# iamarkaj/AwesomeSLAM

Measured on AMD Instinct MI355X. Metric: EKF/UKF filter-steps/s @ N_landmarks, higher is better.
Workload: dtype f32

## Files before the change

### awesomeslam_amd/csrc/aslam_core.hip

```cpp
#include "../../include/aslam_core.h"
#include "../../include/aslam_scan.h"
#include "../../include/aslam_snapshot.h"

#include <hip/hip_runtime.h>

#include <cmath>
#include <cstdio>
#include <cstring>
#include <cstdlib>
#include <algorithm>
#include <mutex>
#include <string>
#include <type_traits>
#include <vector>

#include "ekf_small.h"
#include "ekf_large.h"
#include "ekf_large_launch.h"
#include "scan_front.h"
#include "snapshot.h"
#if ASLAM_HAVE_UKF
#include "ukf_small.h"
#include "ukf_large.h"
#include "ukf_large_launch.h"
// ... 1355 lines not shown
        if (chol_resident)
                *chol_resident = c->large && c->lh.last_resident;
        if (launches_per_callback)
                *launches_per_callback = c->large ? c->lh.last_launches : 1;
        return ASLAM_OK;
}

int aslam_kernel_info(aslam_ctx *c, char *name, int name_cap, int *grid, int *block, int *lds_bytes)
{
        if (!c)
                return fail(ASLAM_ERR_ARG, "null context");
        char buf[192];
        size_t lds = 0;
        if (c->large)
        {
                const LargePlan plan = large_plan(c->cfg.dtype == ASLAM_F32, c->NP, c->cfg.batch, c->cfg.batch, c->lh.knobs);
#if ASLAM_HAVE_UKF
                if (c->cfg.filter == ASLAM_UKF)
                        std::snprintf(buf, sizeof(buf), "ukf_large_wabt + large_update_panel<double> + large_syrk<double> (%d-launch chain per callback, 1 stream)",
                                      ukf_large_plan(c->NP).launches);
                else
#endif
                if (plan.chain == LargeChain::F32_RESIDENT)
                        std::snprintf(buf, sizeof(buf), "%s + %s + large_syrk_bf16x3 (%d-launch chain per callback, %d stream groups)",
                                      plan.chol16 ? "large_chol_bf16" : "large_chol_resident", plan.trsm16 ? "large_trsm_bf16" : "large_trsm_pipe<17>",
                                      plan.launches, c->lh.knobs.groups);
                else if (plan.chain == LargeChain::F32_RIGHT)
                        std::snprintf(buf, sizeof(buf), "large_right_step + large_syrk_bf16x3 (%d-launch chain per callback: one right-looking launch per block column)", plan.launches);
                else if (plan.chain == LargeChain::F32_LEFT)
                        std::snprintf(buf, sizeof(buf), "large_trsm_pipe<17> + large_syrk_bf16x3 (%d-launch chain per callback: multi-workgroup Cholesky)", plan.launches);
                else
                        std::snprintf(buf, sizeof(buf), "large_update_panel<double> (%d-launch chain per callback, %d stream groups)", plan.launches, c->lh.knobs.groups);
                lds = LargeLds::bytes(c->NP);
        }
        else if (c->cfg.filter == ASLAM_EKF)
        {
                std::snprintf(buf, sizeof(buf), "ekf_small_kernel<%d,0>", c->NT);
                lds = with_NT(c->NT, [](auto nt) -> size_t { return SmallLayout<decltype(nt)::value>::total; });
        }
#if ASLAM_HAVE_UKF
        else
        {
                std::snprintf(buf, sizeof(buf), "ukf_small_kernel<%d,0>", c->NT);
                lds = with_NT(c->NT, [](auto nt) -> size_t { return UkfLayout<decltype(nt)::value>::total; });
        }
#endif
        if (name && name_cap > 0)
        {
                std::strncpy(name, buf, name_cap - 1);
// ... 13 lines not shown
```

### awesomeslam_amd/csrc/ekf_large.h

```cpp
#pragma once

#include <type_traits>

#include "small_common.h"

namespace aslam
{
constexpr int LB = 64;
constexpr int LARGE_OBS_CAP = 1024;
constexpr int LARGE_WAIT_CAP = 2048;
constexpr int LARGE_NP_MAX = 1088;
constexpr int LARGE_NB_MAX = LARGE_NP_MAX / LB;

template <typename T> struct LargeView
{
        int NP;
        double *P;
        T *G;
        T *S;
        double *Hc;
        double *Y;
        T *Linv;
        T *Vw;
        unsigned short *Lpl;
        int xrows;
};

typedef float f4 __attribute__((ext_vector_type(4)));
template <typename T> struct Mfma;
template <> struct Mfma<double>
{
        typedef d4 acc_t;
        static __device__ __forceinline__ acc_t zero()
        {
                return (acc_t){0.0, 0.0, 0.0, 0.0};
        }
        static __device__ __forceinline__ acc_t mma(double a, double b, acc_t c)
        {
                return __builtin_amdgcn_mfma_f64_16x16x4f64(a, b, c, 0, 0, 0);
        }
        static __device__ __forceinline__ int row(int lane, int r)
        {
                return (lane >> 4) + 4 * r;
        }
};
template <> struct Mfma<float>
{
        typedef f4 acc_t;
// ... 37 lines not shown
        __host__ __device__ unsigned short *block(int b, int NP, int k, int j) const { return Lq(b, NP) + (size_t)(64 * k) * NP + 64 * j; }
};
template <typename T, typename F> void for_each_array(LargeView<T> &v, F &&f)
{
        const size_t np = (size_t)v.NP;
        f(v.P, np * np, false);
        f(v.G, np * np, true);
        f(v.S, np * np, true);
        f(v.Hc, (np / 2) * 4, false);
        f(v.Y, np, false);
        f(v.Linv, (size_t)LARGE_NB_MAX * LB * LB, false);
        f(v.Lpl, LPlanes::per_filter(v.NP), false);
        f(v.Vw, np * np, true);
}

__host__ __device__ __forceinline__ int lplane_pos(int c)
{
        return 32 * (c >> 5) + 8 * ((c >> 2) & 3) + 4 * ((c >> 4) & 1) + (c & 3);
}

__host__ __device__ __forceinline__ int large_blocks(int n, int xrows = 1)
{
        return (n + xrows + LB - 1) / LB;
}

struct LargeLds
{
        static __host__ __device__ size_t bytes(int NP)
        {
                size_t o = 0;
                o += 8 * (size_t)NP * 2;
                o += 4 * (size_t)LARGE_OBS_CAP * 6;
                o += 4 * (size_t)LARGE_WAIT_CAP * 5;
                o += 4 * (size_t)(NP / 2);
                o += 4 * (size_t)LARGE_OBS_CAP * 4 * 2;
                o += 4 * (size_t)NP;
                o = (o + 15) & ~(size_t)15;
                return o + sizeof(SmallShared);
        }
        static __device__ __forceinline__ SmallLds carve(unsigned char *smem, int NP)
        {
                SmallLds L;
                unsigned char *p = smem;
                L.Lt = nullptr;
                L.Dinv = nullptr;
                L.sY = nullptr;
// ... 151 lines not shown

constexpr int GS_ROW_PAIRS = 2;

template <typename T> __global__ __launch_bounds__(256) void large_build_GS(DevView d, LargeView<T> lv, const int *skipped)
{
        const int b = blockIdx.y;
        if (skipped[b])
                return;
        const int n = d.n[b], NP = lv.NP;
        const int na = large_blocks(n) * LB;
        const int nl = (n - 3) / 2;
        const double *P = lv.P + (size_t)b * NP * NP;
        T *G = lv.G + (size_t)b * NP * NP;
        T *S = lv.S + (size_t)b * NP * NP;
        const double *Hc = lv.Hc + (size_t)b * (NP / 2) * 4;
        const aslam_params *const prm = d.prm + b;
        const double r_xy = prm->r_xy, r_yaw = prm->r_yaw, r_range = prm->r_range, r_bearing = prm->r_bearing;
        const int tid = threadIdx.x;
        const bool pose = (blockIdx.x == 0);
        constexpr int RP = GS_ROW_PAIRS;
        const int r0 = pose ? 0 : 3 + 2 * RP * ((int)blockIdx.x - 1);
        if (r0 >= na)
                return;
        int nlive = 0;
        if (!pose)
        {
                for (int rp = 0; rp < RP; ++rp)
                {
                        const int ra = r0 + 2 * rp;
                        if (ra >= na)
                                break;
                        if (ra < n)
                        {
                                nlive = rp + 1;
                                continue;
                        }
                        for (int rr = ra; rr < min(ra + 2, na); ++rr)
                        {
                                T *grow = G + (size_t)rr * NP, *srow = S + (size_t)rr * NP;
                                const double *Y = lv.Y + (size_t)b * NP;
                                for (int c = tid; c < na; c += 256)
                                {
                                        grow[c] = (rr == n && c < n) ? (T)Y[c] : (T)0;
                                        srow[c] = (c == rr) ? (T)1 : (T)0;
                                }
                        }
                }
                if (nlive == 0)
                        return;
        }
        const double *p0 = P, *p1 = P + NP, *p2 = P + 2 * (size_t)NP;
        const double t00 = p0[0], t01 = p0[1], t02 = p0[2], t10 = p1[0], t11 = p1[1], t12 = p1[2], t20 = p2[0], t21 = p2[1], t22 = p2[2];
        const double *pa[RP], *pb[RP];
        double ta0[RP], ta1[RP], ta2[RP], tb0[RP], tb1[RP], tb2[RP], ha0[RP], ha1[RP], hb0[RP], hb1[RP];
#pragma unroll
        for (int rp = 0; rp < RP; ++rp)
        {
                const int ra = min(r0 + 2 * rp, n - 2);
                pa[rp] = P + (size_t)ra * NP, pb[rp] = pa[rp] + NP;
                ta0[rp] = ta1[rp] = ta2[rp] = tb0[rp] = tb1[rp] = tb2[rp] = ha0[rp] = ha1[rp] = hb0[rp] = hb1[rp] = 0.0;
                if (!pose && rp < nlive)
                {
                        ta0[rp] = pa[rp][0], ta1[rp] = pa[rp][1], ta2[rp] = pa[rp][2];
                        tb0[rp] = pb[rp][0], tb1[rp] = pb[rp][1], tb2[rp] = pb[rp][2];
                        const double *hr = Hc + 4 * ((ra - 3) >> 1);
                        ha0[rp] = hr[0], ha1[rp] = hr[1], hb0[rp] = hr[2], hb1[rp] = hr[3];
// ... 11 lines not shown
                return v - ha * ga - hb * gb;
        };
        if (tid < 3)
        {
                const int c = tid;
                const double g0 = p0[c], g1 = p1[c], g2 = p2[c];
                if (pose)
                {
                        G[c] = (T)g0, G[NP + c] = (T)g1, G[2 * (size_t)NP + c] = (T)g2;
                        S[c] = (T)(g0 + (c == 0 ? r_xy : 0.0));
                        S[NP + c] = (T)(g1 + (c == 1 ? r_xy : 0.0));
                        S[2 * (size_t)NP + c] = (T)(g2 + (c == 2 ? r_yaw : 0.0));
                }
                else
                {
#pragma unroll
                        for (int rp = 0; rp < RP; ++rp)
                                if (rp < nlive)
                                {
                                        const int ra = r0 + 2 * rp;
                                        const double ga = pa[rp][c], gb = pb[rp][c];
                                        G[(size_t)ra * NP + c] = (T)ga;
                                        G[(size_t)(ra + 1) * NP + c] = (T)gb;
                                        S[(size_t)ra * NP + c] = (T)srow(ha0[rp], ha1[rp], false, g0, g1, g2, ga, gb);
                                        S[(size_t)(ra + 1) * NP + c] = (T)srow(hb0[rp], hb1[rp], true, g0, g1, g2, ga, gb);
                                }
                }
        }
        for (int j = tid; j < nl; j += 256)
        {
                const int ce = 3 + 2 * j, co = ce + 1;
                const double h00 = Hc[4 * j], h01 = Hc[4 * j + 1], h10 = Hc[4 * j + 2], h11 = Hc[4 * j + 3];
                double g0e, g0o, g1e, g1o, g2e, g2o;
                grow(h00, h01, h10, h11, t00, t01, t02, p0[ce], p0[co], g0e, g0o);
                grow(h00, h01, h10, h11, t10, t11, t12, p1[ce], p1[co], g1e, g1o);
                grow(h00, h01, h10, h11, t20, t21, t22, p2[ce], p2[co], g2e, g2o);
                if (pose)
                {
                        G[ce] = (T)g0e, G[co] = (T)g0o;
                        G[NP + ce] = (T)g1e, G[NP + co] = (T)g1o;
                        G[2 * (size_t)NP + ce] = (T)g2e, G[2 * (size_t)NP + co] = (T)g2o;
                        if (ce < LB)
                        {
                                S[ce] = (T)g0e, S[co] = (T)g0o;
                                S[NP + ce] = (T)g1e, S[NP + co] = (T)g1o;
                                S[2 * (size_t)NP + ce] = (T)g2e, S[2 * (size_t)NP + co] = (T)g2o;
                        }
                }
                else
                {
#pragma unroll
                        for (int rp = 0; rp < RP; ++rp)
                                if (rp < nlive)
                                {
                                        const int ra = r0 + 2 * rp;
                                        double gae, gao, gbe, gbo;
                                        grow(h00, h01, h10, h11, ta0[rp], ta1[rp], ta2[rp], pa[rp][ce], pa[rp][co], gae, gao);
                                        grow(h00, h01, h10, h11, tb0[rp], tb1[rp], tb2[rp], pb[rp][ce], pb[rp][co], gbe, gbo);
                                        T *ga = G + (size_t)ra * NP, *gb = ga + NP, *sa = S + (size_t)ra * NP, *sb = sa + NP;
                                        ga[ce] = (T)gae, ga[co] = (T)gao;
                                        gb[ce] = (T)gbe, gb[co] = (T)gbo;
                                        if (ce < LB * ((ra + 1) / LB + 1))
                                        {
                                                double se = srow(ha0[rp], ha1[rp], false, g0e, g1e, g2e, gae, gbe),
                                                       so = srow(ha0[rp], ha1[rp], false, g0o, g1o, g2o, gao, gbo);
                                                double ue = srow(hb0[rp], hb1[rp], true, g0e, g1e, g2e, gae, gbe),
                                                       uo = srow(hb0[rp], hb1[rp], true, g0o, g1o, g2o, gao, gbo);
                                                if (ce == ra)
                                                        se += r_range;
                                                if (co == ra + 1)
                                                        uo += r_bearing;
                                                sa[ce] = (T)se, sa[co] = (T)so;
                                                sb[ce] = (T)ue, sb[co] = (T)uo;
                                        }
                                }
                }
        }
        const int nrows = pose ? 3 : 2 * nlive;
        for (int idx = tid; idx < nrows * (na - n); idx += 256)
        {
                const int rr = r0 + idx / (na - n), c = n + idx % (na - n);
                G[(size_t)rr * NP + c] = (T)0;
                S[(size_t)rr * NP + c] = (T)0;
        }
}

struct GsTilesLds
{
        static constexpr int HB = LB + 2, PLD = HB + 1;
        double Pt[HB][PLD];
        double tI[HB][4], tJ[LB][4];
        double cI[HB][2], cJ[LB][2];
        double P3[3][HB], G3[3][LB], P33[3][4];
};
template <typename T> __global__ __launch_bounds__(256) void large_build_GS_tiles(DevView d, LargeView<T> lv, const int *skipped)
{
// ... 10 lines not shown
        const int b = blockIdx.y;
        if (skipped[b])
                return;
        const int n = d.n[b], NP = lv.NP;
        const int nb = large_blocks(n);
        const int tl = blockIdx.x;
        int I = (int)((sqrtf(8.0f * (float)tl + 1.0f) - 1.0f) * 0.5f);
        while ((I + 1) * (I + 2) / 2 <= tl)
                ++I;
        while (I * (I + 1) / 2 > tl)
                --I;
        const int J = tl - I * (I + 1) / 2;
        if (I >= nb)
                return;
        const double *P = lv.P + (size_t)b * NP * NP;
        T *G = lv.G + (size_t)b * NP * NP;
        T *S = lv.S + (size_t)b * NP * NP;
        const double *Hc = lv.Hc + (size_t)b * (NP / 2) * 4;
        const double *Y = lv.Y + (size_t)b * NP;
        const aslam_params *const prm = d.prm + b;
        const double r_xy = prm->r_xy, r_yaw = prm->r_yaw, r_range = prm->r_range, r_bearing = prm->r_bearing;
        const int tid = threadIdx.x;
        const int r0 = LB * I - 1, c0 = LB * J - 1;
        typedef double d2 __attribute__((ext_vector_type(2)));
        {
                const int q = tid & 31, rr = tid >> 5;
#pragma unroll
                for (int ps = 0; ps < (HB + 7) / 8; ++ps)
                {
                        const int r = 8 * ps + rr, gr = r0 + r;
                        if (r < HB)
                        {
                                d2 v = {0.0, 0.0};
                                if (gr >= 0 && gr < NP)
                                        v = *reinterpret_cast<const d2 *>(P + (size_t)gr * NP + LB * J + 2 * q);
                                Pt[r][1 + 2 * q] = v[0], Pt[r][2 + 2 * q] = v[1];
                        }
                }
                if (tid < 2 * HB)
                {
                        const int r = tid >> 1, hc = (tid & 1) ? HB - 1 : 0;
                        const int gr = r0 + r, gc = c0 + hc;
                        Pt[r][hc] = (gr >= 0 && gr < NP && gc >= 0 && gc < NP) ? P[(size_t)gr * NP + gc] : 0.0;
                }
        }
        if (tid < HB)
// ... 40 lines not shown
        const double uJ = cJ[c][0], vJ = cJ[c][1];
        if (rq < 3)
        {
                const int m = rq;
                G3[m][c] = gc >= n ? 0.0 : gc < 3 ? P33[m][gc] : gcol(ceven, uJ, vJ, P33[m][0], P33[m][1], P33[m][2], P3[m][co], P3[m][co + 1]);
        }
        __syncthreads();
        auto g_at = [&](int r) -> double {
                const int ga = r0 + r;
                if (ga < 0 || ga > n || gc >= n)
                        return 0.0;
                if (ga == n)
                        return Y[gc];
                if (gc < 3)
                        return Pt[r][c + 1];
                return gcol(ceven, uJ, vJ, tI[r][0], tI[r][1], tI[r][2], Pt[r][co], Pt[r][co + 1]);
        };
        const double g30 = G3[0][c], g31 = G3[1][c], g32 = G3[2][c];
#pragma unroll 4
        for (int ps = 0; ps < LB / 4; ++ps)
        {
                const int r = 4 * ps + rq, gr = LB * I + r;
                const double g = g_at(r + 1);
                G[(size_t)gr * NP + gc] = (T)g;
                double sv;
                if (gr >= n)
                        sv = (gr == gc) ? 1.0 : 0.0;
                else if (gc >= n)
                        sv = 0.0;
                else if (gr < 3)
                        sv = g + (gr == gc ? (gr < 2 ? r_xy : r_yaw) : 0.0);
                else
                {
                        const bool even = !(gr & 1);
                        const double gp = g_at(even ? r : r + 2);
                        const double go_ = even ? gp : g, ge_ = even ? g : gp;
                        const double ha = cI[r + 1][0], hb = cI[r + 1][1];
                        double v = ha * g30 + hb * g31;
                        if (even)
                                v -= g32;
                        sv = v - ha * go_ - hb * ge_;
                        if (gr == gc)
                                sv += even ? r_bearing : r_range;
                }
                S[(size_t)gr * NP + gc] = (T)sv;
        }
        if (I != J)
        {
                const int a = c, gcolx = LB * I + a;
                const bool even = !(gcolx & 1);
                const int ao = even ? a : a + 1;
                const double uI = cI[a + 1][0], vI = cI[a + 1][1];
#pragma unroll 4
                for (int ps = 0; ps < LB / 4; ++ps)
                {
                        const int cr = 4 * ps + rq, grow = LB * J + cr;
                        double g;
                        if (grow > n || gcolx >= n)
                                g = 0.0;
                        else if (grow == n)
                                g = Y[gcolx];
                        else
                                g = gcol(even, uI, vI, tJ[cr][0], tJ[cr][1], tJ[cr][2], Pt[ao][cr + 1], Pt[ao + 1][cr + 1]);
                        G[(size_t)grow * NP + gcolx] = (T)g;
                }
        }
}


template <typename T> __device__ __forceinline__ T *stacked_row(const LargeView<T> &lv, int b, int na, int vr)
{
        const size_t NP = lv.NP;
        return (vr < na) ? lv.S + ((size_t)b * NP + vr) * NP : lv.G + ((size_t)b * NP + (vr - na)) * NP;
}

template <typename T>
__global__ __launch_bounds__(256) void large_update_panel(DevView d, LargeView<T> lv, int k0, int s_only, const int *skipped)
{
        typedef Mfma<T> MM;
        constexpr int KC = (sizeof(T) == 4) ? 64 : 32;
        constexpr int LD = KC + (sizeof(T) == 4 ? 8 : 4);
        typedef T vec_t __attribute__((ext_vector_type(16 / sizeof(T))));
        constexpr int VW = 16 / sizeof(T);
        static_assert(KC / VW == 16, "16 lanes per staged row");
        __shared__ __attribute__((aligned(16))) T As[2 * LB][LD];
        __shared__ __attribute__((aligned(16))) T Bs[LB][LD];
        const int b = blockIdx.z;
// ... 576 lines not shown
        typedef T vec_t __attribute__((ext_vector_type(16 / sizeof(T))));
        constexpr int VW = 16 / sizeof(T);
        for (int j = VW * lane; j < n; j += 64 * VW)
        {
                const vec_t v = *reinterpret_cast<const vec_t *>(vrow + j), w = *reinterpret_cast<const vec_t *>(q + j);
#pragma unroll
                for (int e = 0; e < VW; ++e)
                        acc = fma((double)v[e], (double)w[e], acc);
        }
        acc = wave_sum_dpp(acc);
        if (lane == 63)
        {
                const double xa = d.X[(size_t)b * NP + a] + acc;
                d.X[(size_t)b * NP + a] = xa;
                if (MODE == MODE_REPLAY)
                {
                        if (a < 3 && poses_out)
                                poses_out[((size_t)b * nsteps + s) * 3 + a] = xa;
                        if (a == 0 && dims_out)
                                dims_out[(size_t)b * nsteps + s] = n;
                }
        }
}
template <int MODE>
__device__ __forceinline__ void x_update_rows_body(float (*sh)[LARGE_NP_MAX], const DevView &d, const LargeView<float> &lv, int b, int xb, int n, int s, int nsteps,
                                                   double *poses_out, int32_t *dims_out)
{
        const int NP = lv.NP;
        const int tid = threadIdx.x, lane = tid & 63;
        if (xb * 4 * XU_ROWS >= n)
                return;
        const float *G = lv.G + (size_t)b * NP * NP;
        for (int j = 4 * tid; j < NP; j += 4 * 256)
        {
                *reinterpret_cast<f4 *>(&sh[0][j]) = *reinterpret_cast<const f4 *>(G + (size_t)n * NP + j);
                *reinterpret_cast<f4 *>(&sh[1][j]) = *reinterpret_cast<const f4 *>(G + j);
                *reinterpret_cast<f4 *>(&sh[2][j]) = *reinterpret_cast<const f4 *>(G + NP + j);
                *reinterpret_cast<f4 *>(&sh[3][j]) = *reinterpret_cast<const f4 *>(G + 2 * (size_t)NP + j);
        }
        __syncthreads();
        double *P = lv.P + (size_t)b * NP * NP;
        const int a0 = (xb * 4 + (tid >> 6)) * XU_ROWS;
        constexpr int NPASS = 5;
        auto load_row = [&](f4 (&v)[NPASS], int a) {
                const float *vr = G + (size_t)min(a, n - 1) * NP;
#pragma unroll
                for (int i = 0; i < NPASS; ++i)
                {
                        const int j = 4 * lane + 256 * i;
                        v[i] = j < n ? *reinterpret_cast<const f4 *>(vr + j) : (f4){0.f, 0.f, 0.f, 0.f};
                }
        };
        f4 vn[NPASS];
        load_row(vn, a0);
#pragma unroll 1
        for (int r = 0; r < XU_ROWS; ++r)
        {
                const int a = a0 + r;
                if (a >= n)
                        break;
                f4 v[NPASS];
#pragma unroll
                for (int i = 0; i < NPASS; ++i)
                        v[i] = vn[i];
                if (r + 1 < XU_ROWS)
                        load_row(vn, a + 1);
                double acc = 0.0, dd = 0.0, d0 = 0.0, d1 = 0.0, d2 = 0.0;
#pragma unroll
                for (int i = 0; i < NPASS; ++i)
                {
                        const int j = 4 * lane + 256 * i;
                        if (j >= n)
                                continue;
                        const f4 wi = *reinterpret_cast<const f4 *>(&sh[0][j]), p0 = *reinterpret_cast<const f4 *>(&sh[1][j]),
                                 p1 = *reinterpret_cast<const f4 *>(&sh[2][j]), p2 = *reinterpret_cast<const f4 *>(&sh[3][j]);
#pragma unroll
                        for (int e = 0; e < 4; ++e)
                        {
                                const double ve = (double)v[i][e];
                                acc = fma(ve, (double)wi[e], acc);
                                dd = fma(ve, ve, dd);
                                d0 = fma(ve, (double)p0[e], d0);
                                d1 = fma(ve, (double)p1[e], d1);
                                d2 = fma(ve, (double)p2[e], d2);
                        }
                }
                acc = wave_sum_dpp(acc), dd = wave_sum_dpp(dd), d0 = wave_sum_dpp(d0), d1 = wave_sum_dpp(d1), d2 = wave_sum_dpp(d2);
                if (lane == 63)
                {
                        double *prow = P + (size_t)a * NP;
                        const double dp[3] = {d0, d1, d2};
                        for (int j = 0; j < 3 && j < a; ++j)
                        {
                                const double pn = prow[j] - dp[j];
                                prow[j] = pn;
                                P[(size_t)j * NP + a] = pn;
                        }
                        prow[a] -= dd;
                        const double xa = d.X[(size_t)b * NP + a] + acc;
                        d.X[(size_t)b * NP + a] = xa;
                        if (MODE == MODE_REPLAY)
                        {
                                if (a < 3 && poses_out)
                                        poses_out[((size_t)b * nsteps + s) * 3 + a] = xa;
                                if (a == 0 && dims_out)
                                        dims_out[(size_t)b * nsteps + s] = n;
                        }
                }
        }
}

template <int MODE>
__global__ __launch_bounds__(256) void large_x_update_rows(DevView d, LargeView<float> lv, int s, int nsteps, double *poses_out, int32_t *dims_out, const int *skipped)
{
        __shared__ __attribute__((aligned(16))) float sh[4][LARGE_NP_MAX];
        const int b = blockIdx.y;
        if (skipped[b])
                return;
        x_update_rows_body<MODE>(sh, d, lv, b, (int)blockIdx.x, d.n[b], s, nsteps, poses_out, dims_out);
}

template <typename T>
__global__ __launch_bounds__(256) void large_stats(DevView d, LargeView<T> lv, int s, int nsteps, StatsView sv, const int *skipped)
{
        __shared__ double red[4][4];
        const int b = blockIdx.x, tid = threadIdx.x, lane = tid & 63;
        if (skipped[b])
        {
                stats_skip(sv, b, s, nsteps, tid);
                return;
        }
        const int n = d.n[b], NP = lv.NP;
        const bool ukf = lv.xrows == 2;
        const T *q = lv.G + ((size_t)b * NP + n) * NP, *t = q + NP;
        const T *Li = lv.Linv + (size_t)b * LARGE_NB_MAX * LB * LB;
        double tt = 0.0, qq = 0.0, qt = 0.0, ld = 0.0;
        for (int j0 = 0; j0 < NP; j0 += 256)
        {
                const int j = j0 + tid;
                const bool in = j < n;
                const int jc = in ? j : 0;
                const double qv = in ? (double)q[jc] : 0.0;
// ... 35 lines not shown
```

### awesomeslam_amd/csrc/ekf_large_launch.h

```cpp
#pragma once

#include <hip/hip_runtime.h>

#include <algorithm>
#include <cstdlib>

#include "ekf_large.h"
#include "aslam_large16.h"

namespace aslam
{
constexpr int LARGE_GROUPS_MAX = 8;
constexpr int CHOL_RESIDENT_MIN_BATCH = 32;

struct LargeKnobs
{
        int groups = 3;
        int chol_resident = -1;
        int right_step = 1;
        int bf16_pipe = 3;
        int keep_l32 = 0;
        int gs_tiles = 0;
        int syrk_running = 0;
};

inline LargeKnobs large_knobs_from_env()
{
        LargeKnobs k;
        auto flag = [](const char *name, int &v) { if (const char *e = std::getenv(name)) v = std::atoi(e) != 0; };
        if (const char *e = std::getenv("ASLAM_LARGE_GROUPS"))
                k.groups = std::max(1, std::min(LARGE_GROUPS_MAX, std::atoi(e)));
        if (const char *e = std::getenv("ASLAM_BF16_PIPE"))
                k.bf16_pipe = std::atoi(e) & 3;
        flag("ASLAM_CHOL_RESIDENT", k.chol_resident);
        flag("ASLAM_RIGHT_STEP", k.right_step);
        flag("ASLAM_KEEP_L32", k.keep_l32);
        flag("ASLAM_GS_TILES", k.gs_tiles);
        flag("ASLAM_SYRK_RUNNING", k.syrk_running);
        return k;
}

enum class LargeChain
{
        F64_LEFT,
        F32_RESIDENT,
        F32_RIGHT,
        F32_LEFT
};

struct LargePlan
{
        LargeChain chain;
        bool chol16, trsm16;
        bool chol_f32out;
        bool gs_tiles, syrk_running;
        int launches;
        bool need_Lpl, need_Vw;
};

inline LargePlan large_plan(bool f32, int NP, int batch, int filters, const LargeKnobs &k)
{
        const int NB = NP / LB;
        auto resident = [&k](int nf) { return k.chol_resident >= 0 ? k.chol_resident != 0 : nf >= CHOL_RESIDENT_MIN_BATCH; };
        LargePlan p = {};
        p.gs_tiles = k.gs_tiles != 0;
        p.syrk_running = k.syrk_running != 0;
        p.need_Lpl = f32 && k.bf16_pipe != 0;
        p.need_Vw = f32 && k.right_step && !resident(batch);
        if (!f32)
                p.chain = LargeChain::F64_LEFT, p.launches = 4 + 2 * NB;
        else if (resident(filters))
        {
                p.chain = LargeChain::F32_RESIDENT, p.launches = 6;
                p.chol16 = (k.bf16_pipe & 2) != 0;
                p.trsm16 = (k.bf16_pipe & 1) != 0;
                p.chol_f32out = !p.trsm16 || k.keep_l32;
        }
        else if (p.need_Vw)
                p.chain = LargeChain::F32_RIGHT, p.launches = 5 + NB;
        else
                p.chain = LargeChain::F32_LEFT, p.launches = 4 + 2 * NB;
        return p;
}

struct LargeHost
{
        LargeKnobs knobs;
        hipStream_t aux[LARGE_GROUPS_MAX - 1] = {};
        hipEvent_t ev_fork = nullptr, ev_join[LARGE_GROUPS_MAX - 1] = {};
        int last_groups = 0;
        int last_launches = 0;
        bool last_resident = false;
};

struct LaunchSlice
{
        int first, count;
        StepArgs sa;
};
// ... 110 lines not shown
                case LargeChain::F32_RESIDENT:
                        if (plan.chol16)
                                launch_chol_bf16(g.dv, g.v, gb, g.skip, g.st, plan.chol_f32out);
                        else
                                hipLaunchKernelGGL(large_chol_resident<LARGE_NB_MAX>, dim3(gb), dim3(256), 0, g.st, g.dv, g.v, g.skip);
                        if (plan.trsm16)
                                launch_trsm_bf16(g.dv, g.v, gb, g.skip, g.st);
                        else
                                hipLaunchKernelGGL(large_trsm_pipe<LARGE_NB_MAX>, dim3(8 * ((gb + 7) / 8) * NB), dim3(256), 0, g.st, g.dv, g.v, gb, g.skip);
                        break;
                case LargeChain::F32_RIGHT:
                        hipLaunchKernelGGL(large_potrf_inv_tiles<T>, dim3(gb), dim3(256), 0, g.st, g.dv, g.v, 0, g.skip);
                        for (int k = 0; k < NB; ++k)
                        {
                                const int M = NB - k - 1;
                                hipLaunchKernelGGL(large_right_step<0>, dim3(M * (M + 1) / 2 + NB * M + NB, 1, gb), dim3(256), 0, g.st, g.dv, g.v, k, g.skip);
                        }
                        vv.G = g.v.Vw;
                        break;
                default:
                        launch_left_looking(g.dv, g.v, NB, gb, g.skip, g.st, 1, false);
                        hipLaunchKernelGGL(large_trsm_pipe<LARGE_NB_MAX>, dim3(8 * ((gb + 7) / 8) * NB), dim3(256), 0, g.st, g.dv, g.v, gb, g.skip);
                }
                if (plan.syrk_running)
                        hipLaunchKernelGGL((large_syrk_bf16x3<true>), syrk_grid, dim3(256), 0, g.st, g.dv, vv, gb, g.skip);
                else
                        hipLaunchKernelGGL((large_syrk_bf16x3<false>), syrk_grid, dim3(256), 0, g.st, g.dv, vv, gb, g.skip);
                hipLaunchKernelGGL((large_x_update_rows<MODE>), dim3((NP + 4 * XU_ROWS - 1) / (4 * XU_ROWS), gb), dim3(256), 0, g.st, g.dv, vv, s, nsteps, g.poses,
                                   g.dims, g.skip);
                if (g.sv.any())
                        hipLaunchKernelGGL(large_stats<T>, dim3(gb), dim3(256), 0, g.st, g.dv, vv, s, nsteps, g.sv, g.skip);
        }
}

template <int MODE, typename T>
hipError_t launch_large(LargeHost &h, const DevView &dv, const LargeView<T> &lv, int *skipped, int64_t t0, int nsteps, double *poses, int32_t *dims,
                        StepArgs sa, hipStream_t st, StatsView sv = {})
{
        const size_t lds = LargeLds::bytes(dv.NP);
        if (hipError_t e = hipFuncSetAttribute(reinterpret_cast<const void *>(large_frontend_kernel<T, MODE>), hipFuncAttributeMaxDynamicSharedMemorySize, (int)lds))
                return e;
        const LaunchSlice sl = launch_slice<MODE>(sa, dv.B);
        const int first = sl.first, Bz = sl.count;
        const LargePlan plan = large_plan(sizeof(T) == 4, dv.NP, dv.B, Bz, h.knobs);
        const bool split = Bz >= std::max(32, 8 * h.knobs.groups);
        const int NG = split ? h.knobs.groups : 1;
        const int per = split ? ((Bz + NG - 1) / NG + 7) & ~7 : Bz;
        LargeGroup<T> g[LARGE_GROUPS_MAX];
        h.last_launches = plan.launches + (sv.any() ? 1 : 0);
        h.last_resident = plan.chain == LargeChain::F32_RESIDENT;
        h.last_groups = 0;
        for (int q = 0; q < NG; ++q)
        {
                const int o = std::min(q * per, Bz);
                const size_t b0 = (size_t)(first + o);
                g[q] = {shifted_dev(dv, b0, MODE == MODE_REPLAY), shifted(lv, b0), skipped + b0, poses, dims, std::min(per, Bz - o), q == 0 ? st : h.aux[q - 1], shifted_stats(sv, b0, nsteps)};
                if (MODE == MODE_REPLAY && poses)
                        g[q].poses += b0 * (size_t)nsteps * 3;
                if (MODE == MODE_REPLAY && dims)
                        g[q].dims += b0 * (size_t)nsteps;
                h.last_groups += g[q].nb > 0;
        }
        hipError_t e = split ? hipEventRecord(h.ev_fork, st) : hipSuccess;
        for (int q = 1; q < NG && e == hipSuccess; ++q)
                e = hipStreamWaitEvent(h.aux[q - 1], h.ev_fork, 0);
        if (e != hipSuccess)
                return e;
        for (int s = 0; s < nsteps; ++s)
                for (int q = 0; q < NG; ++q)
                        if (g[q].nb > 0)
                                launch_large_chain<T, MODE>(plan, g[q], lds, t0, s, nsteps, sl.sa);
        for (int q = 1; q < NG && e == hipSuccess; ++q)
                if ((e = hipEventRecord(h.ev_join[q - 1], h.aux[q - 1])) == hipSuccess)
                        e = hipStreamWaitEvent(st, h.ev_join[q - 1], 0);
        return e != hipSuccess ? e : hipGetLastError();
}
}
```

### awesomeslam_amd/csrc/ekf_large_trsm16.h

```cpp
#pragma once

namespace aslam
{
namespace t16
{
typedef unsigned u4v __attribute__((ext_vector_type(4)));
typedef unsigned u2v __attribute__((ext_vector_type(2)));
typedef __bf16 bf8 __attribute__((ext_vector_type(8)));
typedef __bf16 bf2 __attribute__((ext_vector_type(2)));
typedef float f2v __attribute__((ext_vector_type(2)));

constexpr int PLD = LB;
constexpr int PLANE = LB * PLD;
constexpr int BLK = 3 * PLANE;
constexpr int NBUF = 5;

typedef LPlanes Planes;
__host__ __device__ __forceinline__ int perm_pos(int c)
{
        return lplane_pos(c);
}

__device__ __forceinline__ void split2(float a, float b, unsigned &h, unsigned &m, unsigned &l)
{
// ... 415 lines not shown
        __shared__ __attribute__((aligned(1024))) unsigned short lds[NBUF][BLK];
        __shared__ __attribute__((aligned(1024))) float gl[4][16 * LB];
        const int NP = lv.NP, nblk = NP / LB;
        const int slot = blockIdx.x >> 3;
        const int b = (slot / nblk) * 8 + (blockIdx.x & 7), rb = slot % nblk;
        if (b >= nfilters || skipped[b])
                return;
        const int n = d.n[b];
        const int nb = large_blocks(n);
        if (rb >= nb)
                return;
        const int tid = threadIdx.x, wave = tid >> 6, lane = tid & 63, li = lane & 15, lg = lane >> 4;
        const int wv = __builtin_amdgcn_readfirstlane(wave);
        Rows rows;
        rows.rsrc = __builtin_amdgcn_make_buffer_rsrc(uniform_ptr(lv.G + (size_t)b * NP * NP), 0, NP * NP * 4, 0x00020000);
        rows.so0 = (unsigned)((LB * rb + 16 * wv) * NP * 4);
        rows.out = lv.G + (size_t)b * NP * NP + (size_t)(LB * rb + 16 * wave + li) * NP + 4 * lg;
        rows.rq = rows.rsrc, rows.vq = 0, rows.qplane = 0;
        asm volatile("" ::: "a0", "a255");
        Pipe pp;
        Regs R;
        f4 c[4];
        asm volatile("; ASLAM_STRIP_LIVE_BEGIN vmem: global_store_dwordx4=4" ::: "memory");
        sweep16<STAMP, false>(c, R, pp, lds, gl[wv], pl, b, nb, nb, NP, rows, tid);
        asm volatile("; ASLAM_STRIP_LIVE_END" ::: "memory");
        if constexpr (STAMP)
                if (tid == 0 && blockIdx.x == 0)
                        for (int i = 0; i < 13; ++i)
                                lv.Y[i] = (double)pp.ph[i];
}

template <int NBMAX, bool F32OUT = true>
__global__ __launch_bounds__(256, 1) void large_chol_bf16(DevView d, LargeView<float> lv, t16::Planes pl, const int *skipped)
{
        using namespace t16;
        static_assert(NBMAX == 17, "the chain lists 17 block columns");
        constexpr int PIPE_BYTES = NBUF * BLK * 2, TILE_BYTES = chol64::TILES * TSZ * (int)sizeof(double);
        static_assert(TILE_BYTES <= PIPE_BYTES, "the tiles of the diagonal factorisation alias the block buffers");
        __shared__ __attribute__((aligned(1024))) unsigned short lds[NBUF][BLK];
        __shared__ __attribute__((aligned(1024))) float gl[4][16 * LB];
        double *tiles = reinterpret_cast<double *>(&lds[0][0]);
        const int b = blockIdx.x;
        if (skipped[b])
                return;
        const int n = d.n[b], NP = lv.NP;
        const int nb = large_blocks(n);
        const int tid0 = threadIdx.x;
        const int wv = __builtin_amdgcn_readfirstlane(tid0 >> 6);
        float *Sb = lv.S + (size_t)b * NP * NP;
        float *Linv = lv.Linv + (size_t)b * LARGE_NB_MAX * LB * LB;
        asm volatile("" ::: "a0", "a255");
        Rows rows;
        rows.rsrc = __builtin_amdgcn_make_buffer_rsrc(uniform_ptr(Sb), 0, NP * NP * 4, 0x00020000);
        rows.rq = __builtin_amdgcn_make_buffer_rsrc(uniform_ptr(pl.Lq(b, NP)), 0, 3 * NP * NP * 2, 0x00020000);
        rows.qplane = (unsigned)(NP * NP * 2);
        bool ok = true;
        Pipe pp;
        Regs R;
#pragma unroll 1
        for (int I = 0; I < nb; ++I)
        {
                int tid = tid0;
                asm volatile("" : "+v"(tid));
                const int wave = tid >> 6, lane = tid & 63, li = lane & 15, lg = lane >> 4;
                rows.so0 = (unsigned)((LB * I + 16 * wv) * NP * 4);
                rows.out = Sb + (size_t)(LB * I + 16 * wave + li) * NP + 4 * lg;
                rows.vq = (unsigned)(((LB * I + 16 * wave + li) * NP + 8 * lg) * 2);
                f4 c[4];
                if constexpr (F32OUT)
                        asm volatile("; ASLAM_STRIP_LIVE_BEGIN vmem: global_store_dwordx4=4 buffer_store_dwordx4=6" ::: "memory");
                else
                        asm volatile("; ASLAM_STRIP_LIVE_BEGIN vmem: buffer_store_dwordx4=6" ::: "memory");
                sweep16<false, true, F32OUT>(c, R, pp, lds, gl[wv], pl, b, I, nb, NP, rows, tid);
                asm volatile("; ASLAM_STRIP_LIVE_END" ::: "memory");
                asm volatile("s_waitcnt vmcnt(0)\n\ts_barrier" ::: "memory");
#pragma unroll
                for (int t = 0; t < 4; ++t)
                {
                        if (t <= wave)
                        {
                                double *T = chol64::Lt(tiles, wave, t) + li * TLD + 4 * lg;
#pragma unroll
                                for (int r = 0; r < 4; ++r)
                                        T[r] = (double)c[t][r];
                        }
                }
                ok = chol64::factor_and_invert<true>(tiles, tid) && ok;
                chol64::store_block(tiles, Sb + ((size_t)LB * I) * NP + (size_t)LB * I, NP, Linv + (size_t)I * LB * LB, tid, pl.block(b, NP, I, I));
                asm volatile("s_waitcnt vmcnt(0)" ::: "memory");
                __syncthreads();
        }
        if (!ok && tid0 == 0)
                atomicOr(&d.status[b], 4u);
}

template <int UNUSED = 0>
// ... 39 lines not shown
```

Before: 37370.

## Handle small trailing Cholesky border analytically instead of a full extra block column

When the augmented matrix size leaves only 1 or 3 rows past a multiple of 64, the blocked bf16 Cholesky and TRSM now stop at the last full block. The leftover 3x3 border is factored inside the x-update kernel from dot products of the saved G rows, and a Linv block is written for it. The goal is to skip a whole 64-wide block-column sweep in the chol/trsm chain for these sizes. In exchange the Jacobian kernels do extra scattered writes, the x-update does extra reductions, and the x-update launch moves ahead of syrk, which adds ordering and correctness risk.

After: 38220 (median of 6 runs). 1.02x the previous value.

```diff
diff --git a/awesomeslam_amd/csrc/aslam_core.hip b/awesomeslam_amd/csrc/aslam_core.hip
--- a/awesomeslam_amd/csrc/aslam_core.hip
+++ b/awesomeslam_amd/csrc/aslam_core.hip
@@ -1401,9 +1401,9 @@
                 else
 #endif
                 if (plan.chain == LargeChain::F32_RESIDENT)
-                        std::snprintf(buf, sizeof(buf), "%s + %s + large_syrk_bf16x3 (%d-launch chain per callback, %d stream groups)",
+                        std::snprintf(buf, sizeof(buf), "%s + %s + large_syrk_bf16x3%s (%d-launch chain per callback, %d stream groups)",
                                       plan.chol16 ? "large_chol_bf16" : "large_chol_resident", plan.trsm16 ? "large_trsm_bf16" : "large_trsm_pipe<17>",
-                                      plan.launches, c->lh.knobs.groups);
+                                      plan.border ? " + border" : "", plan.launches, c->lh.knobs.groups);
                 else if (plan.chain == LargeChain::F32_RIGHT)
                         std::snprintf(buf, sizeof(buf), "large_right_step + large_syrk_bf16x3 (%d-launch chain per callback: one right-looking launch per block column)", plan.launches);
                 else if (plan.chain == LargeChain::F32_LEFT)
diff --git a/awesomeslam_amd/csrc/ekf_large.h b/awesomeslam_amd/csrc/ekf_large.h
--- a/awesomeslam_amd/csrc/ekf_large.h
+++ b/awesomeslam_amd/csrc/ekf_large.h
@@ -24,6 +24,7 @@
         T *Vw;
         unsigned short *Lpl;
         int xrows;
+        int border;
 };
 
 typedef float f4 __attribute__((ext_vector_type(4)));
@@ -107,6 +108,24 @@
 __host__ __device__ __forceinline__ int large_blocks(int n, int xrows = 1)
 {
         return (n + xrows + LB - 1) / LB;
+}
+
+struct LargeBorder
+{
+        int t;
+        int nbc;
+};
+__host__ __device__ __forceinline__ LargeBorder large_border(int n, int enabled)
+{
+        const int n0 = n & ~(LB - 1), t = n - n0;
+        const bool on = enabled && n0 >= LB && (t == 1 || t == 3);
+        return {on ? t : 0, on ? n0 / LB : large_blocks(n)};
+}
+constexpr int BORDER_MAX = 3;
+constexpr int BORDER_SAVE = 8, BORDER_SAVE_ROWS = 4;
+__host__ __device__ __forceinline__ bool border_spare(const LargeBorder &bd, int n, int row, int col)
+{
+        return bd.t && row > n && row <= n + bd.t && (col < LB * bd.nbc || (col >= LB * bd.nbc + BORDER_SAVE && col < LB * bd.nbc + BORDER_SAVE + BORDER_SAVE_ROWS));
 }
 
 struct LargeLds
@@ -304,6 +323,16 @@
         const int r0 = pose ? 0 : 3 + 2 * RP * ((int)blockIdx.x - 1);
         if (r0 >= na)
                 return;
+        const LargeBorder bd = large_border(n, lv.border);
+        const int n0 = LB * bd.nbc;
+        auto put_l = [&](int r, int c, double v) {
+                if (bd.t && r >= n0 && c < n0)
+                        G[(size_t)(r + bd.t + 1) * NP + c] = (T)v;
+        };
+        auto save_g2 = [&](int m, int c, T v) {
+                if (bd.t && c >= n0 && c < n)
+                        G[(size_t)(n + 1 + c - n0) * NP + n0 + BORDER_SAVE + m] = v;
+        };
         int nlive = 0;
         if (!pose)
         {
@@ -323,7 +352,10 @@
                                 const double *Y = lv.Y + (size_t)b * NP;
                                 for (int c = tid; c < na; c += 256)
                                 {
-                                        grow[c] = (rr == n && c < n) ? (T)Y[c] : (T)0;
+                                        if (!border_spare(bd, n, rr, c))
+                                                grow[c] = (rr == n && c < n) ? (T)Y[c] : (T)0;
+                                        if (rr == n)
+                                                save_g2(3, c, (T)Y[c]);
                                         srow[c] = (c == rr) ? (T)1 : (T)0;
                                 }
                         }
@@ -381,8 +413,10 @@
                                         const double ga = pa[rp][c], gb = pb[rp][c];
                                         G[(size_t)ra * NP + c] = (T)ga;
                                         G[(size_t)(ra + 1) * NP + c] = (T)gb;
-                                        S[(size_t)ra * NP + c] = (T)srow(ha0[rp], ha1[rp], false, g0, g1, g2, ga, gb);
-                                        S[(size_t)(ra + 1) * NP + c] = (T)srow(hb0[rp], hb1[rp], true, g0, g1, g2, ga, gb);
+                                        const double sa = srow(ha0[rp], ha1[rp], false, g0, g1, g2, ga, gb), sb = srow(hb0[rp], hb1[rp], true, g0, g1, g2, ga, gb);
+                                        S[(size_t)ra * NP + c] = (T)sa;
+                                        S[(size_t)(ra + 1) * NP + c] = (T)sb;
+                                        put_l(ra, c, sa), put_l(ra + 1, c, sb);
                                 }
                 }
         }
@@ -399,6 +433,9 @@
                         G[ce] = (T)g0e, G[co] = (T)g0o;
                         G[NP + ce] = (T)g1e, G[NP + co] = (T)g1o;
                         G[2 * (size_t)NP + ce] = (T)g2e, G[2 * (size_t)NP + co] = (T)g2o;
+                        save_g2(0, ce, (T)g0e), save_g2(0, co, (T)g0o);
+                        save_g2(1, ce, (T)g1e), save_g2(1, co, (T)g1o);
+                        save_g2(2, ce, (T)g2e), save_g2(2, co, (T)g2o);
                         if (ce < LB)
                         {
                                 S[ce] = (T)g0e, S[co] = (T)g0o;
@@ -431,6 +468,8 @@
                                                         uo += r_bearing;
                                                 sa[ce] = (T)se, sa[co] = (T)so;
                                                 sb[ce] = (T)ue, sb[co] = (T)uo;
+                                                put_l(ra, ce, se), put_l(ra, co, so);
+                                                put_l(ra + 1, ce, ue), put_l(ra + 1, co, uo);
                                         }
                                 }
                 }
@@ -487,6 +526,12 @@
         const double r_xy = prm->r_xy, r_yaw = prm->r_yaw, r_range = prm->r_range, r_bearing = prm->r_bearing;
         const int tid = threadIdx.x;
         const int r0 = LB * I - 1, c0 = LB * J - 1;
+        const LargeBorder bd = large_border(n, lv.border);
+        const int n0 = LB * bd.nbc;
+        auto save_g2 = [&](int m, int c_, T v) {
+                if (bd.t && c_ >= n0 && c_ < n)
+                        G[(size_t)(n + 1 + c_ - n0) * NP + n0 + BORDER_SAVE + m] = v;
+        };
         typedef double d2 __attribute__((ext_vector_type(2)));
         {
                 const int q = tid & 31, rr = tid >> 5;
@@ -573,7 +618,10 @@
         {
                 const int r = 4 * ps + rq, gr = LB * I + r;
                 const double g = g_at(r + 1);
-                G[(size_t)gr * NP + gc] = (T)g;
+                if (!border_spare(bd, n, gr, gc))
+                        G[(size_t)gr * NP + gc] = (T)g;
+                if (gr == n)
+                        save_g2(3, gc, (T)g);
                 double sv;
                 if (gr >= n)
                         sv = (gr == gc) ? 1.0 : 0.0;
@@ -595,6 +643,8 @@
                                 sv += even ? r_bearing : r_range;
                 }
                 S[(size_t)gr * NP + gc] = (T)sv;
+                if (bd.t && gr >= n0 && gr < n && gc < n0)
+                        G[(size_t)(gr + bd.t + 1) * NP + gc] = (T)sv;
         }
         if (I != J)
         {
@@ -614,6 +664,8 @@
                         else
                                 g = gcol(even, uI, vI, tJ[cr][0], tJ[cr][1], tJ[cr][2], Pt[ao][cr + 1], Pt[ao + 1][cr + 1]);
                         G[(size_t)grow * NP + gcolx] = (T)g;
+                        if (grow < 3)
+                                save_g2(grow, gcolx, (T)g);
                 }
         }
 }
@@ -1236,37 +1288,152 @@
                 }
         }
 }
-template <int MODE>
-__device__ __forceinline__ void x_update_rows_body(float (*sh)[LARGE_NP_MAX], const DevView &d, const LargeView<float> &lv, int b, int xb, int n, int s, int nsteps,
-                                                   double *poses_out, int32_t *dims_out)
+constexpr int XU_SH_ROWS = 4 + BORDER_MAX;
+constexpr int XU_NDOT = 4 * BORDER_MAX + BORDER_MAX * (BORDER_MAX + 1) / 2;
+
+struct XuBorder
+{
+        double Li[BORDER_MAX][BORDER_MAX];
+        float v2[4][BORDER_MAX];
+        bool ok;
+};
+
+__device__ __forceinline__ XuBorder x_update_border(float (*sh)[LARGE_NP_MAX], double (*red)[XU_NDOT], const LargeView<float> &lv, int b, int n, const LargeBorder &bd)
+{
+        constexpr int BM = BORDER_MAX;
+        const int NP = lv.NP, tid = threadIdx.x, t = bd.t, n0 = LB * bd.nbc;
+        const float *G = lv.G + (size_t)b * NP * NP, *S = lv.S + (size_t)b * NP * NP;
+        float s22[BM][BM], g2[4][BM];
+#pragma unroll
+        for (int i = 0; i < BM; ++i)
+#pragma unroll
+                for (int j = 0; j <= i; ++j)
+                        s22[i][j] = i < t ? S[(size_t)(n0 + i) * NP + n0 + j] : (i == j ? 1.f : 0.f);
+#pragma unroll
+        for (int k = 0; k < BM; ++k)
+#pragma unroll
+                for (int m = 0; m < 4; ++m)
+                        g2[m][k] = k < t ? G[(size_t)(n + 1 + k) * NP + n0 + BORDER_SAVE + ((m + 3) & 3)] : 0.f;
+        double dot[XU_NDOT];
+#pragma unroll
+        for (int i = 0; i < XU_NDOT; ++i)
+                dot[i] = 0.0;
+        for (int j = 4 * tid; j < n0; j += 4 * 256)
+        {
+                f4 r[XU_SH_ROWS];
+                r[0] = *reinterpret_cast<const f4 *>(G + (size_t)n * NP + j);
+#pragma unroll
+                for (int m = 0; m < 3; ++m)
+                        r[1 + m] = *reinterpret_cast<const f4 *>(G + (size_t)m * NP + j);
+#pragma unroll
+                for (int k = 0; k < BM; ++k)
+                        r[4 + k] = k < t ? *reinterpret_cast<const f4 *>(G + (size_t)(n + 1 + k) * NP + j) : (f4){0.f, 0.f, 0.f, 0.f};
+#pragma unroll
+                for (int m = 0; m < XU_SH_ROWS; ++m)
+                        *reinterpret_cast<f4 *>(&sh[m][j]) = r[m];
+#pragma unroll
+                for (int e = 0; e < 4; ++e)
+                {
+#pragma unroll
+                        for (int m = 0; m < 4; ++m)
+#pragma unroll
+                                for (int k = 0; k < BM; ++k)
+                                        dot[BM * m + k] = fma((double)r[m][e], (double)r[4 + k][e], dot[BM * m + k]);
+#pragma unroll
+                        for (int i = 0; i < BM; ++i)
+#pragma unroll
+                                for (int k = 0; k <= i; ++k)
+                                        dot[4 * BM + i * (i + 1) / 2 + k] = fma((double)r[4 + i][e], (double)r[4 + k][e], dot[4 * BM + i * (i + 1) / 2 + k]);
+                }
+        }
+#pragma unroll
+        for (int i = 0; i < XU_NDOT; ++i)
+                dot[i] = wave_sum_dpp(dot[i]);
+        if ((tid & 63) == 63)
+        {
+#pragma unroll
+                for (int i = 0; i < XU_NDOT; ++i)
+                        red[tid >> 6][i] = dot[i];
+        }
+        __syncthreads();
+#pragma unroll
+        for (int i = 0; i < XU_NDOT; ++i)
+                dot[i] = (red[0][i] + red[1][i]) + (red[2][i] + red[3][i]);
+        XuBorder bx;
+        double L[BM][BM];
+        bx.ok = true;
+#pragma unroll
+        for (int j = 0; j < BM; ++j)
+        {
+                double sjj = (double)s22[j][j] - dot[4 * BM + j * (j + 1) / 2 + j];
+#pragma unroll
+                for (int k = 0; k < j; ++k)
+                        sjj -= L[j][k] * L[j][k];
+                bx.ok = bx.ok && sjj > 0.0;
+                L[j][j] = sqrt(sjj);
+#pragma unroll
+                for (int i = j + 1; i < BM; ++i)
+                {
+                        double sij = (double)s22[i][j] - dot[4 * BM + i * (i + 1) / 2 + j];
+#pragma unroll
+                        for (int k = 0; k < j; ++k)
+                                sij -= L[i][k] * L[j][k];
+                        L[i][j] = sij / L[j][j];
+                }
+        }
+        static_assert(BM == 3, "the inverse below is written out for 3 x 3");
+        bx.Li[0][0] = 1.0 / L[0][0], bx.Li[1][1] = 1.0 / L[1][1], bx.Li[2][2] = 1.0 / L[2][2];
+        bx.Li[1][0] = -(L[1][0] * bx.Li[0][0]) * bx.Li[1][1];
+        bx.Li[2][1] = -(L[2][1] * bx.Li[1][1]) * bx.Li[2][2];
+        bx.Li[2][0] = -(L[2][0] * bx.Li[0][0] + L[2][1] * bx.Li[1][0]) * bx.Li[2][2];
+        bx.Li[0][1] = bx.Li[0][2] = bx.Li[1][2] = 0.0;
+#pragma unroll
+        for (int m = 0; m < 4; ++m)
+#pragma unroll
+                for (int j = 0; j < BM; ++j)
+                {
+                        double v = 0.0;
+#pragma unroll
+                        for (int k = 0; k <= j; ++k)
+                                v += ((double)g2[m][k] - dot[BM * m + k]) * bx.Li[j][k];
+                        bx.v2[m][j] = (float)v;
+                }
+        return bx;
+}
+
+template <int MODE, bool BORDER>
+__device__ __forceinline__ void x_update_rows_loop(const float (*sh)[LARGE_NP_MAX], const XuBorder &bx, const DevView &d, const LargeView<float> &lv, int b, int xb, int n,
+                                                   int n0, int s, int nsteps, double *poses_out, int32_t *dims_out)
 {
         const int NP = lv.NP;
         const int tid = threadIdx.x, lane = tid & 63;
-        if (xb * 4 * XU_ROWS >= n)
-                return;
-        const float *G = lv.G + (size_t)b * NP * NP;
-        for (int j = 4 * tid; j < NP; j += 4 * 256)
-        {
-                *reinterpret_cast<f4 *>(&sh[0][j]) = *reinterpret_cast<const f4 *>(G + (size_t)n * NP + j);
-                *reinterpret_cast<f4 *>(&sh[1][j]) = *reinterpret_cast<const f4 *>(G + j);
-                *reinterpret_cast<f4 *>(&sh[2][j]) = *reinterpret_cast<const f4 *>(G + NP + j);
-                *reinterpret_cast<f4 *>(&sh[3][j]) = *reinterpret_cast<const f4 *>(G + 2 * (size_t)NP + j);
-        }
-        __syncthreads();
+        float *G = lv.G + (size_t)b * NP * NP;
         double *P = lv.P + (size_t)b * NP * NP;
         const int a0 = (xb * 4 + (tid >> 6)) * XU_ROWS;
         constexpr int NPASS = 5;
-        auto load_row = [&](f4 (&v)[NPASS], int a) {
+        const int jlim = BORDER ? n0 : n;
+        auto load_row = [&](f4 (&v)[NPASS], f4 &g2, int a) {
                 const float *vr = G + (size_t)min(a, n - 1) * NP;
 #pragma unroll
                 for (int i = 0; i < NPASS; ++i)
                 {
                         const int j = 4 * lane + 256 * i;
-                        v[i] = j < n ? *reinterpret_cast<const f4 *>(vr + j) : (f4){0.f, 0.f, 0.f, 0.f};
-                }
+                        v[i] = j < jlim ? *reinterpret_cast<const f4 *>(vr + j) : (f4){0.f, 0.f, 0.f, 0.f};
+                }
+                if constexpr (BORDER)
+                        g2 = *reinterpret_cast<const f4 *>(vr + n0);
         };
-        f4 vn[NPASS];
-        load_row(vn, a0);
+        float pv[3][BORDER_MAX];
+#pragma unroll
+        for (int m = 0; m < 3; ++m)
+#pragma unroll
+                for (int k = 0; k < BORDER_MAX; ++k)
+                {
+                        pv[m][k] = bx.v2[1 + m][k];
+                        asm volatile("" : "+v"(pv[m][k]));
+                }
+        f4 vn[NPASS], g2n = {0.f, 0.f, 0.f, 0.f};
+        load_row(vn, g2n, a0);
 #pragma unroll 1
         for (int r = 0; r < XU_ROWS; ++r)
         {
@@ -1274,20 +1441,24 @@
                 if (a >= n)
                         break;
                 f4 v[NPASS];
+                const f4 g2 = g2n;
 #pragma unroll
                 for (int i = 0; i < NPASS; ++i)
                         v[i] = vn[i];
                 if (r + 1 < XU_ROWS)
-                        load_row(vn, a + 1);
-                double acc = 0.0, dd = 0.0, d0 = 0.0, d1 = 0.0, d2 = 0.0;
+                        load_row(vn, g2n, a + 1);
+                double acc = 0.0, dd = 0.0, d0 = 0.0, d1 = 0.0, d2 = 0.0, e0 = 0.0, e1 = 0.0, e2 = 0.0;
 #pragma unroll
                 for (int i = 0; i < NPASS; ++i)
                 {
                         const int j = 4 * lane + 256 * i;
-                        if (j >= n)
+                        if (j >= jlim)
                                 continue;
                         const f4 wi = *reinterpret_cast<const f4 *>(&sh[0][j]), p0 = *reinterpret_cast<const f4 *>(&sh[1][j]),
                                  p1 = *reinterpret_cast<const f4 *>(&sh[2][j]), p2 = *reinterpret_cast<const f4 *>(&sh[3][j]);
+                        f4 l0 = {0.f, 0.f, 0.f, 0.f}, l1 = l0, l2 = l0;
+                        if constexpr (BORDER)
+                                l0 = *reinterpret_cast<const f4 *>(&sh[4][j]), l1 = *reinterpret_cast<const f4 *>(&sh[5][j]), l2 = *reinterpret_cast<const f4 *>(&sh[6][j]);
 #pragma unroll
                         for (int e = 0; e < 4; ++e)
                         {
@@ -1297,11 +1468,43 @@
                                 d0 = fma(ve, (double)p0[e], d0);
                                 d1 = fma(ve, (double)p1[e], d1);
                                 d2 = fma(ve, (double)p2[e], d2);
+                                if constexpr (BORDER)
+                                {
+                                        e0 = fma(ve, (double)l0[e], e0);
+                                        e1 = fma(ve, (double)l1[e], e1);
+                                        e2 = fma(ve, (double)l2[e], e2);
+                                }
                         }
                 }
                 acc = wave_sum_dpp(acc), dd = wave_sum_dpp(dd), d0 = wave_sum_dpp(d0), d1 = wave_sum_dpp(d1), d2 = wave_sum_dpp(d2);
+                if constexpr (BORDER)
+                        e0 = wave_sum_dpp(e0), e1 = wave_sum_dpp(e1), e2 = wave_sum_dpp(e2);
                 if (lane == 63)
                 {
+                        if constexpr (BORDER)
+                        {
+                                const double w0 = (double)g2[0] - e0, w1 = (double)g2[1] - e1, w2 = (double)g2[2] - e2;
+                                float x0 = (float)(w0 * bx.Li[0][0]), x1 = (float)(w0 * bx.Li[1][0] + w1 * bx.Li[1][1]),
+                                      x2 = (float)(w0 * bx.Li[2][0] + w1 * bx.Li[2][1] + w2 * bx.Li[2][2]);
+                                if (a < 3)
+                                {
+                                        x0 = a == 0 ? pv[0][0] : a == 1 ? pv[1][0] : pv[2][0];
+                                        x1 = a == 0 ? pv[0][1] : a == 1 ? pv[1][1] : pv[2][1];
+                                        x2 = a == 0 ? pv[0][2] : a == 1 ? pv[1][2] : pv[2][2];
+                                }
+                                *reinterpret_cast<f4 *>(G + (size_t)a * NP + n0) = (f4){x0, x1, x2, 0.f};
+                                const float xs[BORDER_MAX] = {x0, x1, x2};
+#pragma unroll
+                                for (int k = 0; k < BORDER_MAX; ++k)
+                                {
+                                        const double ve = (double)xs[k];
+                                        acc = fma(ve, (double)bx.v2[0][k], acc);
+                                        dd = fma(ve, ve, dd);
+                                        d0 = fma(ve, (double)bx.v2[1][k], d0);
+                                        d1 = fma(ve, (double)bx.v2[2][k], d1);
+                                        d2 = fma(ve, (double)bx.v2[3][k], d2);
+                                }
+                        }
                         double *prow = P + (size_t)a * NP;
                         const double dp[3] = {d0, d1, d2};
                         for (int j = 0; j < 3 && j < a; ++j)
@@ -1325,13 +1528,65 @@
 }
 
 template <int MODE>
+__device__ __forceinline__ void x_update_rows_body(float (*sh)[LARGE_NP_MAX], double (*red)[XU_NDOT], const DevView &d, const LargeView<float> &lv, int b, int xb, int n,
+                                                   int s, int nsteps, double *poses_out, int32_t *dims_out)
+{
+        const int NP = lv.NP;
+        const int tid = threadIdx.x;
+        if (xb * 4 * XU_ROWS >= n)
+                return;
+        float *G = lv.G + (size_t)b * NP * NP;
+        const LargeBorder bd = large_border(n, lv.border);
+        const int n0 = LB * bd.nbc;
+        XuBorder bx = {};
+        if (bd.t)
+        {
+                bx = x_update_border(sh, red, lv, b, n, bd);
+                if (xb == 0)
+                {
+                        float *Lb = lv.Linv + ((size_t)b * LARGE_NB_MAX + bd.nbc) * LB * LB;
+                        for (int e = tid; e < LB * LB; e += 256)
+                        {
+                                const int r = e >> 6, c = e & (LB - 1);
+                                double v = r == c ? 1.0 : 0.0;
+                                if (r < BORDER_MAX && c <= r)
+                                        v = r == 0 ? bx.Li[0][0] : r == 1 ? (c == 0 ? bx.Li[1][0] : bx.Li[1][1]) : (c == 0 ? bx.Li[2][0] : c == 1 ? bx.Li[2][1] : bx.Li[2][2]);
+                                Lb[e] = (float)v;
+                        }
+                        if (tid == 0)
+                        {
+                                *reinterpret_cast<f4 *>(G + (size_t)n * NP + n0) = (f4){bx.v2[0][0], bx.v2[0][1], bx.v2[0][2], 0.f};
+                                if (!bx.ok)
+                                        atomicOr(&d.status[b], 4u);
+                        }
+                }
+        }
+        else
+        {
+                for (int j = 4 * tid; j < NP; j += 4 * 256)
+                {
+                        *reinterpret_cast<f4 *>(&sh[0][j]) = *reinterpret_cast<const f4 *>(G + (size_t)n * NP + j);
+                        *reinterpret_cast<f4 *>(&sh[1][j]) = *reinterpret_cast<const f4 *>(G + j);
+                        *reinterpret_cast<f4 *>(&sh[2][j]) = *reinterpret_cast<const f4 *>(G + NP + j);
+                        *reinterpret_cast<f4 *>(&sh[3][j]) = *reinterpret_cast<const f4 *>(G + 2 * (size_t)NP + j);
+                }
+                __syncthreads();
+        }
+        if (bd.t)
+                x_update_rows_loop<MODE, true>(sh, bx, d, lv, b, xb, n, n0, s, nsteps, poses_out, dims_out);
+        else
+                x_update_rows_loop<MODE, false>(sh, bx, d, lv, b, xb, n, n0, s, nsteps, poses_out, dims_out);
+}
+
+template <int MODE>
 __global__ __launch_bounds__(256) void large_x_update_rows(DevView d, LargeView<float> lv, int s, int nsteps, double *poses_out, int32_t *dims_out, const int *skipped)
 {
-        __shared__ __attribute__((aligned(16))) float sh[4][LARGE_NP_MAX];
+        __shared__ __attribute__((aligned(16))) float sh[XU_SH_ROWS][LARGE_NP_MAX];
+        __shared__ double red[4][XU_NDOT];
         const int b = blockIdx.y;
         if (skipped[b])
                 return;
-        x_update_rows_body<MODE>(sh, d, lv, b, (int)blockIdx.x, d.n[b], s, nsteps, poses_out, dims_out);
+        x_update_rows_body<MODE>(sh, red, d, lv, b, (int)blockIdx.x, d.n[b], s, nsteps, poses_out, dims_out);
 }
 
 template <typename T>
diff --git a/awesomeslam_amd/csrc/ekf_large_launch.h b/awesomeslam_amd/csrc/ekf_large_launch.h
--- a/awesomeslam_amd/csrc/ekf_large_launch.h
+++ b/awesomeslam_amd/csrc/ekf_large_launch.h
@@ -21,6 +21,7 @@
         int bf16_pipe = 3;
         int keep_l32 = 0;
         int gs_tiles = 0;
+        int border = 1;
         int syrk_running = 0;
 };
 
@@ -37,6 +38,7 @@
         flag("ASLAM_KEEP_L32", k.keep_l32);
         flag("ASLAM_GS_TILES", k.gs_tiles);
         flag("ASLAM_SYRK_RUNNING", k.syrk_running);
+        flag("ASLAM_BORDER", k.border);
         return k;
 }
 
@@ -52,6 +54,7 @@
 {
         LargeChain chain;
         bool chol16, trsm16;
+        bool border;
         bool chol_f32out;
         bool gs_tiles, syrk_running;
         int launches;
@@ -75,6 +78,7 @@
                 p.chol16 = (k.bf16_pipe & 2) != 0;
                 p.trsm16 = (k.bf16_pipe & 1) != 0;
                 p.chol_f32out = !p.trsm16 || k.keep_l32;
+                p.border = p.chol16 && p.trsm16 && !k.keep_l32 && k.border != 0;
         }
         else if (p.need_Vw)
                 p.chain = LargeChain::F32_RIGHT, p.launches = 5 + NB;
@@ -231,12 +235,18 @@
                         launch_left_looking(g.dv, g.v, NB, gb, g.skip, g.st, 1, false);
                         hipLaunchKernelGGL(large_trsm_pipe<LARGE_NB_MAX>, dim3(8 * ((gb + 7) / 8) * NB), dim3(256), 0, g.st, g.dv, g.v, gb, g.skip);
                 }
+                auto x_update = [&]() {
+                        hipLaunchKernelGGL((large_x_update_rows<MODE>), dim3((NP + 4 * XU_ROWS - 1) / (4 * XU_ROWS), gb), dim3(256), 0, g.st, g.dv, vv, s, nsteps,
+                                           g.poses, g.dims, g.skip);
+                };
+                if (plan.border)
+                        x_update();
                 if (plan.syrk_running)
                         hipLaunchKernelGGL((large_syrk_bf16x3<true>), syrk_grid, dim3(256), 0, g.st, g.dv, vv, gb, g.skip);
                 else
                         hipLaunchKernelGGL((large_syrk_bf16x3<false>), syrk_grid, dim3(256), 0, g.st, g.dv, vv, gb, g.skip);
-                hipLaunchKernelGGL((large_x_update_rows<MODE>), dim3((NP + 4 * XU_ROWS - 1) / (4 * XU_ROWS), gb), dim3(256), 0, g.st, g.dv, vv, s, nsteps, g.poses,
-                                   g.dims, g.skip);
+                if (!plan.border)
+                        x_update();
                 if (g.sv.any())
                         hipLaunchKernelGGL(large_stats<T>, dim3(gb), dim3(256), 0, g.st, g.dv, vv, s, nsteps, g.sv, g.skip);
         }
@@ -264,6 +274,7 @@
                 const int o = std::min(q * per, Bz);
                 const size_t b0 = (size_t)(first + o);
                 g[q] = {shifted_dev(dv, b0, MODE == MODE_REPLAY), shifted(lv, b0), skipped + b0, poses, dims, std::min(per, Bz - o), q == 0 ? st : h.aux[q - 1], shifted_stats(sv, b0, nsteps)};
+                g[q].v.border = plan.border;
                 if (MODE == MODE_REPLAY && poses)
                         g[q].poses += b0 * (size_t)nsteps * 3;
                 if (MODE == MODE_REPLAY && dims)
diff --git a/awesomeslam_amd/csrc/ekf_large_trsm16.h b/awesomeslam_amd/csrc/ekf_large_trsm16.h
--- a/awesomeslam_amd/csrc/ekf_large_trsm16.h
+++ b/awesomeslam_amd/csrc/ekf_large_trsm16.h
@@ -461,7 +461,7 @@
         Regs R;
         f4 c[4];
         asm volatile("; ASLAM_STRIP_LIVE_BEGIN vmem: global_store_dwordx4=4" ::: "memory");
-        sweep16<STAMP, false>(c, R, pp, lds, gl[wv], pl, b, nb, nb, NP, rows, tid);
+        sweep16<STAMP, false>(c, R, pp, lds, gl[wv], pl, b, large_border(n, lv.border).nbc, nb, NP, rows, tid);
         asm volatile("; ASLAM_STRIP_LIVE_END" ::: "memory");
         if constexpr (STAMP)
                 if (tid == 0 && blockIdx.x == 0)
@@ -483,7 +483,7 @@
         if (skipped[b])
                 return;
         const int n = d.n[b], NP = lv.NP;
-        const int nb = large_blocks(n);
+        const int nbc = large_border(n, lv.border).nbc;
         const int tid0 = threadIdx.x;
         const int wv = __builtin_amdgcn_readfirstlane(tid0 >> 6);
         float *Sb = lv.S + (size_t)b * NP * NP;
@@ -497,7 +497,7 @@
         Pipe pp;
         Regs R;
 #pragma unroll 1
-        for (int I = 0; I < nb; ++I)
+        for (int I = 0; I < nbc; ++I)
         {
                 int tid = tid0;
                 asm volatile("" : "+v"(tid));
@@ -510,7 +510,7 @@
                         asm volatile("; ASLAM_STRIP_LIVE_BEGIN vmem: global_store_dwordx4=4 buffer_store_dwordx4=6" ::: "memory");
                 else
                         asm volatile("; ASLAM_STRIP_LIVE_BEGIN vmem: buffer_store_dwordx4=6" ::: "memory");
-                sweep16<false, true, F32OUT>(c, R, pp, lds, gl[wv], pl, b, I, nb, NP, rows, tid);
+                sweep16<false, true, F32OUT>(c, R, pp, lds, gl[wv], pl, b, I, nbc, NP, rows, tid);
                 asm volatile("; ASLAM_STRIP_LIVE_END" ::: "memory");
                 asm volatile("s_waitcnt vmcnt(0)\n\ts_barrier" ::: "memory");
 #pragma unroll
```
